# Azure/mmlspark

Hardware: NVIDIA H100
Metric: boosting_iters_per_sec (higher is better)
Workload: dtype int64 fixed-point histograms over u8 bins (fp32 gradients, fp64 split gains)

## Files before the change

mmlspark_b200/csrc/hist_kernel.cuh:

```cuda
#pragma once
#include <cstdint>
#include <cuda_runtime.h>

namespace b200gbm {

constexpr int kTileFeat = 32;
constexpr int kBins = 256;
constexpr int kLoBits = 18;
constexpr int kFlushRows = 1 << (32 - kLoBits);
#ifndef B200GBM_K4_EXPERIMENT
#define B200GBM_K4_EXPERIMENT 0
#endif
#ifndef B200GBM_STAGE_ROWS
#define B200GBM_STAGE_ROWS 512
#endif
#ifndef B200GBM_STAGES
#define B200GBM_STAGES 3
#endif
#ifndef B200GBM_HIST_THREADS
#define B200GBM_HIST_THREADS 512
#endif
constexpr int kStageRows = B200GBM_STAGE_ROWS;
constexpr int kStages = B200GBM_STAGES;
constexpr int kHistThreads = B200GBM_HIST_THREADS;
constexpr int kStageSlots = (kStageRows * 2 + kHistThreads - 1) / kHistThreads;
constexpr int kHistWarps = kHistThreads / 32;
constexpr int kPlaneWords = kBins * kTileFeat;
constexpr int kHistSmemBytes =
    4 * kPlaneWords * 4 + kStages * (kStageRows * 32 + kStageRows * 16);

struct HistWork {
  int begin;
  int count;
  int use_idx;
  int buf;
};

__global__ void __launch_bounds__(256)
k_gather_q(const HistWork* __restrict__ work, const int* __restrict__ idx0, const int* __restrict__ idx1, const int4* __restrict__ qgh,
           int4* __restrict__ qord) {
  const HistWork w = *work;
  if (!w.use_idx) return;
  const int* __restrict__ idx = w.buf ? idx1 : idx0;
  for (int i = blockIdx.x * blockDim.x + threadIdx.x; i < w.count; i += gridDim.x * blockDim.x) {
    const int p = w.begin + i;
    qord[p] = qgh[idx[p]];
  }
}


__device__ __forceinline__ void cp_async16(void* smem, const void* gmem, bool valid) {
  unsigned s = static_cast<unsigned>(__cvta_generic_to_shared(smem));
  int sz = valid ? 16 : 0;
  asm volatile("cp.async.cg.shared.global [%0], [%1], 16, %2;\n" ::"r"(s), "l"(gmem), "r"(sz));
}
__device__ __forceinline__ void cp_async_commit() { asm volatile("cp.async.commit_group;\n" ::); }
template <int N>
__device__ __forceinline__ void cp_async_wait() {
  asm volatile("cp.async.wait_group %0;\n" ::"n"(N));
}

template <int NATOM>
__global__ void __launch_bounds__(kHistThreads, 1)
k4_hist_build(const uint8_t* __restrict__ bins, size_t rows_stride, int num_tiles,
              const int4* __restrict__ qgh, const int* __restrict__ idx0, const int* __restrict__ idx1,
              const HistWork* __restrict__ work, unsigned long long* __restrict__ hist) {
  extern __shared__ __align__(16) unsigned char smem_raw[];
  unsigned* plane = reinterpret_cast<unsigned*>(smem_raw);
  unsigned char* stage_bins = smem_raw + 4 * kPlaneWords * 4;
  int4* stage_q = reinterpret_cast<int4*>(stage_bins + kStages * kStageRows * 32);

  const HistWork w = *work;
  const int n = w.count;
  if (n <= 0) return;
  const int tid = threadIdx.x, lane = tid & 31, warp = tid >> 5;
  const int* __restrict__ idx = w.buf ? idx1 : idx0;

  long long cells_rows = static_cast<long long>(n) * num_tiles;
  int rpi = static_cast<int>((cells_rows + gridDim.x - 1) / gridDim.x);
  rpi = max(rpi, 2048);
  rpi = min(rpi, kFlushRows);
  rpi = (rpi + kStageRows - 1) / kStageRows * kStageRows;
  const int chunks = (n + rpi - 1) / rpi;
  const int items = chunks * num_tiles;

  for (int e = tid; e < 4 * kPlaneWords; e += kHistThreads) plane[e] = 0u;
  __syncthreads();

  for (int item = blockIdx.x; item < items; item += gridDim.x) {
    const int tile = item % num_tiles;
    const int chunk = item / num_tiles;
    const int row0 = chunk * rpi;
    const int nrows = min(rpi, n - row0);
    const int nst = (nrows + kStageRows - 1) / kStageRows;
    const uint8_t* tbins = bins + static_cast<size_t>(tile) * rows_stride * 32;

    auto row_of = [&](int st, int slot) -> int {
      int hrow = slot * kHistThreads + tid;
      if (hrow >= kStageRows * 2) return -1;
      int p = row0 + st * kStageRows + (hrow >> 1);
      if (p >= row0 + nrows) return -1;
      return w.use_idx ? idx[w.begin + p] : (w.begin + p);
    };
    auto issue = [&](int st, int slot, int r) {
      int hrow = slot * kHistThreads + tid;
      if (hrow >= kStageRows * 2) return;
      int srow = hrow >> 1, shalf = hrow & 1;
      int buf = st % kStages;
      bool ok = r >= 0;
      size_t rr = ok ? static_cast<size_t>(r) : 0;
      cp_async16(stage_bins + (buf * kStageRows + srow) * 32 + shalf * 16,
                 tbins + rr * 32 + shalf * 16, ok);
      if (shalf == 0) cp_async16(stage_q + buf * kStageRows + srow, qgh + rr, ok);
    };

    int rnext[kStageSlots];
#pragma unroll
    for (int sl = 0; sl < kStageSlots; ++sl) rnext[sl] = row_of(0, sl);
#pragma unroll
    for (int s = 0; s < kStages - 1; ++s) {
      if (s < nst) {
#pragma unroll
        for (int sl = 0; sl < kStageSlots; ++sl) {
          int r = rnext[sl];
          rnext[sl] = (s + 1 < nst) ? row_of(s + 1, sl) : -1;
          issue(s, sl, r);
        }
      }
      cp_async_commit();
    }
    for (int s = 0; s < nst; ++s) {
      cp_async_wait<kStages - 2>();
      __syncthreads();
      int sn = s + kStages - 1;
      if (sn < nst) {
#pragma unroll
        for (int sl = 0; sl < kStageSlots; ++sl) {
          int r = rnext[sl];
          rnext[sl] = (sn + 1 < nst) ? row_of(sn + 1, sl) : -1;
          issue(sn, sl, r);
        }
      }
      cp_async_commit();

      const int buf = s % kStages;
      const unsigned* sw = reinterpret_cast<const unsigned*>(stage_bins + buf * kStageRows * 32);
      const int4* sq = stage_q + buf * kStageRows;
      const int rsel = lane >> 3, wsel = lane & 7;
#pragma unroll 2
      for (int k4 = 0; k4 < kStageRows / (4 * kHistWarps); ++k4) {
        const int r = (warp + k4 * kHistWarps) * 4 + rsel;
        const unsigned word = sw[r * 8 + wsel];
        const int4 q = sq[r];
#pragma unroll
        for (int k = 0; k < 4; ++k) {
          const int kk = (k + rsel) & 3;
          const unsigned b = (word >> (8 * kk)) & 0xFFu;
          const unsigned a = b * 32u + static_cast<unsigned>(wsel * 4 + kk);
          atomicAdd(&plane[a], static_cast<unsigned>(q.x));
          atomicAdd(&plane[kPlaneWords + a], static_cast<unsigned>(q.y));
          atomicAdd(&plane[2 * kPlaneWords + a], static_cast<unsigned>(q.z));
          if (NATOM == 4) atomicAdd(&plane[3 * kPlaneWords + a], static_cast<unsigned>(q.w));
        }
      }
    }
    cp_async_wait<0>();
    __syncthreads();
    for (int e = tid; e < kPlaneWords; e += kHistThreads) {
      unsigned ghi = plane[e], glo = plane[kPlaneWords + e];
      unsigned hhi = plane[2 * kPlaneWords + e];
      unsigned hlo = (NATOM == 4) ? plane[3 * kPlaneWords + e] : 0u;
      if (ghi | glo | hhi | hlo) {
        int f = tile * 32 + (e & 31);
        int b = e >> 5;
        long long g = (static_cast<long long>(static_cast<int>(ghi)) << kLoBits) +
                      static_cast<long long>(glo);
        long long h;
        if (NATOM == 4)
          h = (static_cast<long long>(static_cast<int>(hhi)) << kLoBits) +
              static_cast<long long>(hlo);
        else
          h = static_cast<long long>(hhi);
        size_t o = (static_cast<size_t>(f) * kBins + b) * 2;
        if (g) atomicAdd(&hist[o], static_cast<unsigned long long>(g));
        if (h) atomicAdd(&hist[o + 1], static_cast<unsigned long long>(h));
        plane[e] = 0u;
        plane[kPlaneWords + e] = 0u;
        plane[2 * kPlaneWords + e] = 0u;
        if (NATOM == 4) plane[3 * kPlaneWords + e] = 0u;
      }
    }
    __syncthreads();
  }
}


constexpr int kWsConsumerWarps = 16;
#ifndef B200GBM_WS_PRODUCERS
#define B200GBM_WS_PRODUCERS 2
#endif
constexpr int kWsProducerWarps = B200GBM_WS_PRODUCERS;
constexpr int kWsThreads = (kWsConsumerWarps + kWsProducerWarps) * 32;
constexpr int kWsStageRows = 512;
constexpr int kWsStages = 3;
constexpr int kWsSmemBytes = 4 * kPlaneWords * 4 + kWsStages * (kWsStageRows * 32 + kWsStageRows * 16) + 64;

__device__ __forceinline__ unsigned smem_u32(const void* p) { return static_cast<unsigned>(__cvta_generic_to_shared(p)); }
__device__ __forceinline__ void mbar_init(unsigned long long* bar, unsigned count) {
  asm volatile("mbarrier.init.shared::cta.b64 [%0], %1;\n" ::"r"(smem_u32(bar)), "r"(count));
}
__device__ __forceinline__ void mbar_arrive(unsigned long long* bar) {
  asm volatile("mbarrier.arrive.shared::cta.b64 _, [%0];\n" ::"r"(smem_u32(bar)) : "memory");
}
__device__ __forceinline__ void mbar_arrive_expect_tx(unsigned long long* bar, unsigned bytes) {
  asm volatile("mbarrier.arrive.expect_tx.shared::cta.b64 _, [%0], %1;\n" ::"r"(smem_u32(bar)), "r"(bytes) : "memory");
}
__device__ __forceinline__ void mbar_expect_tx(unsigned long long* bar, unsigned bytes) {
  asm volatile("mbarrier.expect_tx.relaxed.cta.shared::cta.b64 [%0], %1;\n" ::"r"(smem_u32(bar)), "r"(bytes) : "memory");
}
__device__ __forceinline__ void mbar_wait(unsigned long long* bar, unsigned parity) {
  asm volatile(
      "{\n"
      ".reg .pred p;\n"
      "WAIT_LOOP:\n"
      "mbarrier.try_wait.parity.shared::cta.b64 p, [%0], %1;\n"
      "@p bra DONE;\n"
      "bra WAIT_LOOP;\n"
      "DONE:\n"
      "}\n" ::"r"(smem_u32(bar)), "r"(parity) : "memory");
}
__device__ __forceinline__ void tma_bulk_g2s(void* smem_dst, const void* gmem_src, unsigned bytes, unsigned long long* bar) {
  asm volatile("cp.async.bulk.shared::cluster.global.mbarrier::complete_tx::bytes [%0], [%1], %2, [%3];\n" ::"r"(smem_u32(smem_dst)),
               "l"(gmem_src), "r"(bytes), "r"(smem_u32(bar))
               : "memory");
}
__device__ __forceinline__ void cp_async_mbar_arrive_noinc(unsigned long long* bar) {
  asm volatile("cp.async.mbarrier.arrive.noinc.shared::cta.b64 [%0];\n" ::"r"(smem_u32(bar)) : "memory");
}

template <int NATOM>
__global__ void __launch_bounds__(kWsThreads, 1)
k4_hist_build_ws(const uint8_t* __restrict__ bins, size_t rows_stride, int num_tiles, const int4* __restrict__ qgh,
                 const int4* __restrict__ qord, const int* __restrict__ idx0, const int* __restrict__ idx1,
                 const HistWork* __restrict__ work, unsigned long long* __restrict__ hist) {
  extern __shared__ __align__(128) unsigned char smem_raw[];
  unsigned* plane = reinterpret_cast<unsigned*>(smem_raw);
  unsigned char* stage_bins = smem_raw + 4 * kPlaneWords * 4;
  int4* stage_q = reinterpret_cast<int4*>(stage_bins + kWsStages * kWsStageRows * 32);
  unsigned long long* full_bar = reinterpret_cast<unsigned long long*>(reinterpret_cast<unsigned char*>(stage_q) + kWsStages * kWsStageRows * 16);
  unsigned long long* empty_bar = full_bar + kWsStages;

  const HistWork w = *work;
  const int n = w.count;
  if (n <= 0) return;
  const int tid = threadIdx.x, lane = tid & 31, warp = tid >> 5;
  const int* __restrict__ idx = w.buf ? idx1 : idx0;

  long long cells_rows = static_cast<long long>(n) * num_tiles;
  int rpi = static_cast<int>((cells_rows + 4LL * gridDim.x - 1) / (4LL * gridDim.x));
  rpi = (rpi + kWsStageRows - 1) / kWsStageRows * kWsStageRows;
  rpi = max(rpi, kWsStageRows);
  rpi = min(rpi, kFlushRows);
  const int chunks = (n + rpi - 1) / rpi;
  const long long items = static_cast<long long>(chunks) * num_tiles;
  const int i0 = static_cast<int>(items * blockIdx.x / gridDim.x);
  const int i1 = static_cast<int>(items * (blockIdx.x + 1) / gridDim.x);
  if (i0 >= i1) return;

  if (tid == 0) {
    for (int i = 0; i < kWsStages; ++i) { mbar_init(&full_bar[i], kWsProducerWarps * 32); mbar_init(&empty_bar[i], kWsConsumerWarps); }
    asm volatile("fence.mbarrier_init.release.cluster;\n" ::: "memory");
  }
  for (int e = tid; e < 4 * kPlaneWords; e += kWsThreads) plane[e] = 0u;
  __syncthreads();

  unsigned gs = 0;
  if (warp >= kWsConsumerWarps) {
    const int ptid = tid - kWsConsumerWarps * 32;
    constexpr int kPT = kWsProducerWarps * 32;
    constexpr int kPerLane = kWsStageRows / kPT;
    for (int item = i0; item < i1; ++item) {
      const int tile = item / chunks, chunk = item - tile * chunks;
      const int row0 = chunk * rpi;
      const int nrows = min(rpi, n - row0);
      const int nst = (nrows + kWsStageRows - 1) / kWsStageRows;
      const uint8_t* tbins = bins + static_cast<size_t>(tile) * rows_stride * 32;
      for (int s = 0; s < nst; ++s, ++gs) {
        const int slot = gs % kWsStages;
        mbar_wait(&empty_bar[slot], ((gs / kWsStages) & 1u) ^ 1u);
        const int p0 = row0 + s * kWsStageRows;
        const int rows = min(kWsStageRows, row0 + nrows - p0);
        unsigned char* db = stage_bins + slot * kWsStageRows * 32;
        int4* dq = stage_q + slot * kWsStageRows;
        if (!w.use_idx) {
          if (ptid == 0) {
            mbar_arrive_expect_tx(&full_bar[slot], static_cast<unsigned>(rows) * 48u);
            const size_t r = static_cast<size_t>(w.begin + p0);
            tma_bulk_g2s(db, tbins + r * 32, static_cast<unsigned>(rows) * 32u, &full_bar[slot]);
            tma_bulk_g2s(dq, qgh + r, static_cast<unsigned>(rows) * 16u, &full_bar[slot]);
          } else {
            mbar_arrive(&full_bar[slot]);
          }
        } else {
          const int* ip = idx + w.begin + p0;
          if (ptid == 0) {
            mbar_expect_tx(&full_bar[slot], static_cast<unsigned>(rows) * 16u);
            tma_bulk_g2s(dq, qord + static_cast<size_t>(w.begin + p0), static_cast<unsigned>(rows) * 16u, &full_bar[slot]);
          }
          int rr[2 * kPerLane];
#pragma unroll
          for (int k = 0; k < 2 * kPerLane; ++k) { const int j = (ptid + k * kPT) >> 1; rr[k] = j < rows ? ip[j] : -1; }
#pragma unroll
          for (int k = 0; k < 2 * kPerLane; ++k) {
            const int hh = ptid + k * kPT, j = hh >> 1, half = (hh & 1) * 16;
            if (rr[k] >= 0) cp_async16(db + j * 32 + half, tbins + static_cast<size_t>(rr[k]) * 32 + half, true);
          }
          cp_async_mbar_arrive_noinc(&full_bar[slot]);
        }
      }
    }
    cp_async_wait<0>();
  } else {
#if B200GBM_K4_EXPERIMENT != 0
    unsigned exp_sink = 0;
#endif
    const int sub = lane >> 2, rot = lane & 3;
    int acc_rows = 0;
    for (int item = i0; item < i1; ++item) {
      const int tile = item / chunks, chunk = item - tile * chunks;
      const int row0 = chunk * rpi;
      const int nrows = min(rpi, n - row0);
      const int nst = (nrows + kWsStageRows - 1) / kWsStageRows;
      for (int s = 0; s < nst; ++s, ++gs) {
        const int slot = gs % kWsStages;
        mbar_wait(&full_bar[slot], (gs / kWsStages) & 1u);
        const int rows = min(kWsStageRows, nrows - s * kWsStageRows);
        const unsigned* sw = reinterpret_cast<const unsigned*>(stage_bins + slot * kWsStageRows * 32);
        const int4* sq = stage_q + slot * kWsStageRows;
        const int groups = (rows + 31) >> 5;
        for (int g = warp; g < groups; g += kWsConsumerWarps) {
          const int r = g * 32 + lane;
          if (r < rows) {
            const int4 q = sq[r];
            const unsigned* rw = sw + r * 8;
#pragma unroll
            for (int k = 0; k < 8; ++k) {
              const int w8 = (sub + k) & 7;
              const unsigned word = rw[w8];
#pragma unroll
              for (int j = 0; j < 4; ++j) {
                const int kk = (j + rot) & 3;
                const unsigned b = (word >> (8 * kk)) & 0xFFu;
                const unsigned a = b * 32u + static_cast<unsigned>(w8 * 4 + kk);
#if B200GBM_K4_EXPERIMENT == 0
                atomicAdd(&plane[a], static_cast<unsigned>(q.x));
                atomicAdd(&plane[kPlaneWords + a], static_cast<unsigned>(q.y));
                atomicAdd(&plane[2 * kPlaneWords + a], static_cast<unsigned>(q.z));
                if (NATOM == 4) atomicAdd(&plane[3 * kPlaneWords + a], static_cast<unsigned>(q.w));
#else
                if (B200GBM_K4_EXPERIMENT >= 2) atomicAdd(&plane[a], static_cast<unsigned>(q.x));
                if (B200GBM_K4_EXPERIMENT >= 3) atomicAdd(&plane[kPlaneWords + a], static_cast<unsigned>(q.y));
                if (B200GBM_K4_EXPERIMENT == 1) exp_sink ^= a + static_cast<unsigned>(q.x ^ q.y ^ q.z ^ q.w);
#endif
              }
            }
          }
        }
#if B200GBM_K4_EXPERIMENT != 0
        if (exp_sink == 0x12345679u) plane[lane] = exp_sink;
#endif
        __syncwarp();
        if (lane == 0) mbar_arrive(&empty_bar[slot]);
      }
      acc_rows += nrows;
      bool flush = (item + 1 == i1);
      if (!flush) {
        const int ntile = (item + 1) / chunks, nchunk = (item + 1) - ntile * chunks;
        const int nnext = min(rpi, n - nchunk * rpi);
        flush = (ntile != tile) || (acc_rows + nnext > kFlushRows);
      }
      if (!flush) continue;
      acc_rows = 0;
      asm volatile("bar.sync 1, %0;\n" ::"n"(kWsConsumerWarps * 32) : "memory");
      for (int e = tid; e < kPlaneWords; e += kWsConsumerWarps * 32) {
        unsigned ghi = plane[e], glo = plane[kPlaneWords + e];
        unsigned hhi = plane[2 * kPlaneWords + e];
        unsigned hlo = (NATOM == 4) ? plane[3 * kPlaneWords + e] : 0u;
        if (ghi | glo | hhi | hlo) {
          const int f = tile * 32 + (e & 31);
          const int b = e >> 5;
          long long g = (static_cast<long long>(static_cast<int>(ghi)) << kLoBits) + static_cast<long long>(glo);
          long long h = (NATOM == 4) ? (static_cast<long long>(static_cast<int>(hhi)) << kLoBits) + static_cast<long long>(hlo)
                                     : static_cast<long long>(hhi);
          const size_t o = (static_cast<size_t>(f) * kBins + b) * 2;
          if (g) atomicAdd(&hist[o], static_cast<unsigned long long>(g));
          if (h) atomicAdd(&hist[o + 1], static_cast<unsigned long long>(h));
          plane[e] = 0u;
          plane[kPlaneWords + e] = 0u;
          plane[2 * kPlaneWords + e] = 0u;
          if (NATOM == 4) plane[3 * kPlaneWords + e] = 0u;
        }
      }
      asm volatile("bar.sync 1, %0;\n" ::"n"(kWsConsumerWarps * 32) : "memory");
    }
  }
}


}
```

Baseline: 5.151.

## Flush shared histogram planes via bulk async reduce-add instead of per-cell atomics

The flush phase now walks the shared histogram in 32-bin slabs. Each consumer thread packs two (g,h) int64 pairs into a shared staging buffer, and one thread issues cp.reduce.async.bulk add.u64 operations, one per feature row, into global memory. This replaces the scattered per-cell 64-bit global atomics and lets the reductions run asynchronously alongside later work. The cost is an extra staging buffer, a barrier per slab, and full-slab reductions even for zero cells, unless the whole slab is zero. It also adds an experiment mode that skips the flush.

Result: faster. 5.599, median of 6 (+8.7%).

```diff
diff --git a/mmlspark_b200/csrc/hist_kernel.cuh b/mmlspark_b200/csrc/hist_kernel.cuh
--- a/mmlspark_b200/csrc/hist_kernel.cuh
+++ b/mmlspark_b200/csrc/hist_kernel.cuh
@@ -203,7 +203,12 @@
 constexpr int kWsThreads = (kWsConsumerWarps + kWsProducerWarps) * 32;
 constexpr int kWsStageRows = 512;
 constexpr int kWsStages = 3;
-constexpr int kWsSmemBytes = 4 * kPlaneWords * 4 + kWsStages * (kWsStageRows * 32 + kWsStageRows * 16) + 64;
+constexpr int kFlushSlabBins = 32;
+constexpr int kFlushRowBytes = kFlushSlabBins * 16;
+constexpr int kFlushStageBytes = kTileFeat * kFlushRowBytes;
+constexpr int kWsSmemBytes = 4 * kPlaneWords * 4 + kWsStages * (kWsStageRows * 32 + kWsStageRows * 16) + kFlushStageBytes + 64;
+static_assert(kWsSmemBytes <= 227 * 1024, "K4 shared memory exceeds the 227 KB per block of sm_90");
+static_assert(kFlushSlabBins * kTileFeat == 2 * kWsConsumerWarps * 32, "a flush slab is two (g,h) pairs per consumer thread");
 
 __device__ __forceinline__ unsigned smem_u32(const void* p) { return static_cast<unsigned>(__cvta_generic_to_shared(p)); }
 __device__ __forceinline__ void mbar_init(unsigned long long* bar, unsigned count) {
@@ -237,6 +242,15 @@
 __device__ __forceinline__ void cp_async_mbar_arrive_noinc(unsigned long long* bar) {
   asm volatile("cp.async.mbarrier.arrive.noinc.shared::cta.b64 [%0];\n" ::"r"(smem_u32(bar)) : "memory");
 }
+__device__ __forceinline__ void bulk_reduce_add_u64(unsigned long long* gmem_dst, const void* smem_src, unsigned bytes) {
+  asm volatile("cp.reduce.async.bulk.global.shared::cta.bulk_group.add.u64 [%0], [%1], %2;\n" ::"l"(gmem_dst), "r"(smem_u32(smem_src)),
+               "r"(bytes)
+               : "memory");
+}
+__device__ __forceinline__ void bulk_commit() { asm volatile("cp.async.bulk.commit_group;\n" ::: "memory"); }
+__device__ __forceinline__ void bulk_wait_read_all() { asm volatile("cp.async.bulk.wait_group.read 0;\n" ::: "memory"); }
+__device__ __forceinline__ void bulk_wait_all() { asm volatile("cp.async.bulk.wait_group 0;\n" ::: "memory"); }
+__device__ __forceinline__ void fence_proxy_async_smem() { asm volatile("fence.proxy.async.shared::cta;\n" ::: "memory"); }
 
 template <int NATOM>
 __global__ void __launch_bounds__(kWsThreads, 1)
@@ -247,7 +261,8 @@
   unsigned* plane = reinterpret_cast<unsigned*>(smem_raw);
   unsigned char* stage_bins = smem_raw + 4 * kPlaneWords * 4;
   int4* stage_q = reinterpret_cast<int4*>(stage_bins + kWsStages * kWsStageRows * 32);
-  unsigned long long* full_bar = reinterpret_cast<unsigned long long*>(reinterpret_cast<unsigned char*>(stage_q) + kWsStages * kWsStageRows * 16);
+  unsigned char* flush_stage = reinterpret_cast<unsigned char*>(stage_q) + kWsStages * kWsStageRows * 16;
+  unsigned long long* full_bar = reinterpret_cast<unsigned long long*>(flush_stage + kFlushStageBytes);
   unsigned long long* empty_bar = full_bar + kWsStages;
 
   const HistWork w = *work;
@@ -321,7 +336,7 @@
     }
     cp_async_wait<0>();
   } else {
-#if B200GBM_K4_EXPERIMENT != 0
+#if B200GBM_K4_EXPERIMENT >= 1 && B200GBM_K4_EXPERIMENT <= 3
     unsigned exp_sink = 0;
 #endif
     const int sub = lane >> 2, rot = lane & 3;
@@ -352,7 +367,7 @@
                 const int kk = (j + rot) & 3;
                 const unsigned b = (word >> (8 * kk)) & 0xFFu;
                 const unsigned a = b * 32u + static_cast<unsigned>(w8 * 4 + kk);
-#if B200GBM_K4_EXPERIMENT == 0
+#if B200GBM_K4_EXPERIMENT == 0 || B200GBM_K4_EXPERIMENT == 4
                 atomicAdd(&plane[a], static_cast<unsigned>(q.x));
                 atomicAdd(&plane[kPlaneWords + a], static_cast<unsigned>(q.y));
                 atomicAdd(&plane[2 * kPlaneWords + a], static_cast<unsigned>(q.z));
@@ -366,7 +381,7 @@
             }
           }
         }
-#if B200GBM_K4_EXPERIMENT != 0
+#if B200GBM_K4_EXPERIMENT >= 1 && B200GBM_K4_EXPERIMENT <= 3
         if (exp_sink == 0x12345679u) plane[lane] = exp_sink;
 #endif
         __syncwarp();
@@ -382,27 +397,56 @@
       if (!flush) continue;
       acc_rows = 0;
       asm volatile("bar.sync 1, %0;\n" ::"n"(kWsConsumerWarps * 32) : "memory");
-      for (int e = tid; e < kPlaneWords; e += kWsConsumerWarps * 32) {
-        unsigned ghi = plane[e], glo = plane[kPlaneWords + e];
-        unsigned hhi = plane[2 * kPlaneWords + e];
-        unsigned hlo = (NATOM == 4) ? plane[3 * kPlaneWords + e] : 0u;
-        if (ghi | glo | hhi | hlo) {
-          const int f = tile * 32 + (e & 31);
-          const int b = e >> 5;
-          long long g = (static_cast<long long>(static_cast<int>(ghi)) << kLoBits) + static_cast<long long>(glo);
-          long long h = (NATOM == 4) ? (static_cast<long long>(static_cast<int>(hhi)) << kLoBits) + static_cast<long long>(hlo)
-                                     : static_cast<long long>(hhi);
-          const size_t o = (static_cast<size_t>(f) * kBins + b) * 2;
-          if (g) atomicAdd(&hist[o], static_cast<unsigned long long>(g));
-          if (h) atomicAdd(&hist[o + 1], static_cast<unsigned long long>(h));
+      unsigned long long* htile = hist + static_cast<size_t>(tile) * kTileFeat * kBins * 2;
+      int sbin[2];
+#pragma unroll
+      for (int i = 0; i < 2; ++i) sbin[i] = (warp + i * kWsConsumerWarps + lane) & (kFlushSlabBins - 1);
+      for (int b0 = 0; b0 < kBins; b0 += kFlushSlabBins) {
+        long long g[2], h[2];
+        bool nz = false;
+#pragma unroll
+        for (int i = 0; i < 2; ++i) {
+          const int e = (b0 + sbin[i]) * kTileFeat + lane;
+          const unsigned ghi = plane[e], glo = plane[kPlaneWords + e], hhi = plane[2 * kPlaneWords + e];
+          const unsigned hlo = (NATOM == 4) ? plane[3 * kPlaneWords + e] : 0u;
           plane[e] = 0u;
           plane[kPlaneWords + e] = 0u;
           plane[2 * kPlaneWords + e] = 0u;
           if (NATOM == 4) plane[3 * kPlaneWords + e] = 0u;
-        }
-      }
-      asm volatile("bar.sync 1, %0;\n" ::"n"(kWsConsumerWarps * 32) : "memory");
+          nz |= (ghi | glo | hhi | hlo) != 0u;
+          g[i] = (static_cast<long long>(static_cast<int>(ghi)) << kLoBits) + static_cast<long long>(glo);
+          h[i] = (NATOM == 4) ? (static_cast<long long>(static_cast<int>(hhi)) << kLoBits) + static_cast<long long>(hlo)
+                              : static_cast<long long>(hhi);
+        }
+        if (tid == 0) bulk_wait_read_all();
+        asm volatile("bar.sync 1, %0;\n" ::"n"(kWsConsumerWarps * 32) : "memory");
+#pragma unroll
+        for (int i = 0; i < 2; ++i)
+          *reinterpret_cast<longlong2*>(flush_stage + lane * kFlushRowBytes + sbin[i] * 16) = make_longlong2(g[i], h[i]);
+        fence_proxy_async_smem();
+        int any;
+        asm volatile(
+            "{\n"
+            ".reg .pred p, q;\n"
+            "setp.ne.u32 p, %1, 0;\n"
+            "bar.red.or.pred q, 1, %2, p;\n"
+            "selp.s32 %0, 1, 0, q;\n"
+            "}\n"
+            : "=r"(any)
+            : "r"(static_cast<unsigned>(nz)), "n"(kWsConsumerWarps * 32)
+            : "memory");
+#if B200GBM_K4_EXPERIMENT != 4
+        if (tid == 0 && any) {
+          for (int f = 0; f < kTileFeat; ++f)
+            bulk_reduce_add_u64(htile + (static_cast<size_t>(f) * kBins + b0) * 2, flush_stage + f * kFlushRowBytes, kFlushSlabBins * 16);
+          bulk_commit();
+        }
+#else
+        (void)any; (void)htile;
+#endif
+      }
     }
+    if (tid == 0) bulk_wait_all();
   }
 }
 
```
